# MaxHalford/sorobn

Hardware: NVIDIA H100
Metric: exact-inference queries/sec (higher is better)
Workload: dtype f32

## Files before the change

sorobn_b200/csrc/sbn_api.cu:

```cuda
#include <cuda_runtime.h>

#include <algorithm>
#include <cstdarg>
#include <cstdio>
#include <cstdlib>
#include <cstring>
#include <string>
#include <vector>

#include "sbn_chain.h"
#include "sbn_gibbs.cuh"
#include "sbn_internal.h"
#include "sbn_join.h"
#include "sbn_kernels.cuh"
#include "sbn_launch.h"
#include "sbn_pair.h"
#include "sbn_tma.h"

namespace {

thread_local std::string g_err;

int fail(int code, const char *fmt, ...) {
    char buf[512];
// ... 623 lines not shown
            default: return cudaErrorInvalidValue;
        }
        return cudaGetLastError();
    }
    return sbn_batched_launch(q, grid, stream);
}

cudaError_t launch_normalise(sbn_program *P, float *d_out, int64_t ld_out, int64_t n_rows, cudaStream_t stream) {
    P->launches++;
    const int threads = 256;
    const int64_t grid = (n_rows + threads - 1) / threads;
    if (P->f64)
        sbn_normalise<double><<<static_cast<unsigned>(grid), threads, 0, stream>>>(
            reinterpret_cast<const double *>(P->slots[P->post_slot].ptr), P->ld, P->post_batched, P->Q,
            reinterpret_cast<double *>(d_out), ld_out, static_cast<int>(n_rows), 1e-290,
            reinterpret_cast<double *>(P->d_total));
    else
        sbn_normalise<float><<<static_cast<unsigned>(grid), threads, 0, stream>>>(
            P->slots[P->post_slot].ptr, P->ld, P->post_batched, P->Q, d_out, ld_out, static_cast<int>(n_rows),
            SBN_MIN_TOTAL_F32, P->d_total);
    return cudaGetLastError();
}

inline bool hoisted(const sbn_program *P, const StepDesc &st) { return P->mode == 1 && st.kind == 0; }

inline bool chain_on(const sbn_program *P) {
    return P->use_chain && P->chain_fits && P->use_tiled && !P->use_branches && !P->segments.empty();
}

inline bool pair_on(const sbn_program *P) {
    return P->use_pair && P->use_tiled && !P->use_branches && (!chain_on(P) || P->pairs_avoid_segments) && !P->pairs.empty();
}

inline bool graph_allowed(const sbn_program *P) { return P->use_graph; }

int run_table_steps(sbn_program *P) {
    if (P->mode != 1) return SBN_OK;
    SbnStep q;
    for (const StepDesc &st : P->steps) {
        if (!hoisted(P, st)) continue;
        build_params(P, st, nullptr, 0, 1, &q);
        SBN_CUDA(launch_step(P, st, q, P->stream));
    }
    SBN_CUDA(cudaStreamSynchronize(P->stream));
    P->setup_launches = P->launches;
    P->launches = 0;
    return SBN_OK;
}

inline bool fold_normalise(const sbn_program *P, const StepDesc &st, const SbnStep &q) {
#if !SBN_FOLD_NORMALISE
    (void)P;
    (void)st;
    (void)q;
    return false;
#endif
    static const bool enabled = [] {
        const char *e = getenv("SOROBN_B200_FOLD_NORMALISE");
        return e ? atoi(e) != 0 : true;
    }();
    return enabled && !P->f64 && P->post_batched && st.kind == 1 && q.tile_off != nullptr && q.slab_off == nullptr && st.n_tiles == 1 &&
           st.n_out == P->Q && !sbn_tma_eligible(P, st);
}

int issue_all(sbn_program *P, const uint8_t *d_ev, int64_t ld_ev, int64_t n_rows, float *d_out, int64_t ld_out,
              cudaStream_t stream, cudaEvent_t *events) {
    SbnStep q;
    int k = 0;
    bool folded = false;
    bool skip_second = false;
    for (const StepDesc &st : P->steps) {
        if (events) SBN_CUDA(cudaEventRecord(events[k], stream));
        ++k;
        if (hoisted(P, st)) continue;
        const int seg = chain_on(P) ? P->seg_first[k - 1] : -1;
        if (seg == -2) continue;
        if (seg >= 0) {
            P->launches++;
            SBN_CUDA(sbn_chain_launch(P, *P->segments[seg], d_ev, ld_ev, n_rows, d_out, ld_out, stream));
            continue;
        }
        int pair = pair_on(P) ? P->pair_first[k - 1] : -1;
        if (pair == -2 && !skip_second) pair = -1;
        skip_second = false;
        if (pair == -2) continue;
        if (pair >= 0 && !sbn_pair_fits(P, *P->pairs[pair])) pair = -1;
        if (pair >= 0) {
            skip_second = true;
            P->launches++;
            SBN_CUDA(sbn_pair_launch(P, *P->pairs[pair], d_ev, ld_ev, n_rows, stream));
            continue;
        }
        build_params(P, st, d_ev, ld_ev, n_rows, &q);
        if (k == static_cast<int>(P->steps.size()) && fold_normalise(P, st, q)) {
            q.norm_out = d_out;
            q.norm_ld = ld_out;
            q.norm_totals = P->d_total;
            q.norm_min = SBN_MIN_TOTAL_F32;
            folded = true;
        }
        SBN_CUDA(launch_step(P, st, q, stream));
    }
    if (events) SBN_CUDA(cudaEventRecord(events[k], stream));
    if (!folded && !(chain_on(P) && !P->segments.empty() && P->segments.back()->ends_in_posterior))
        SBN_CUDA(launch_normalise(P, d_out, ld_out, n_rows, stream));
    if (events) SBN_CUDA(cudaEventRecord(events[k + 1], stream));
    return SBN_OK;
// ... 72 lines not shown
}

extern "C" {

int sbn_abi_version(void) { return SBN_ABI_VERSION; }
const char *sbn_last_error(void) { return g_err.c_str(); }

int sbn_device_count(int *count) {
    if (!count) return fail(SBN_E_INVALID, "null count");
    int n = 0;
    cudaError_t e = cudaGetDeviceCount(&n);
    if (e != cudaSuccess || n == 0) {
        *count = 0;
        return fail(SBN_E_NODEVICE, "no CUDA device: %s", cudaGetErrorString(e));
    }
    *count = n;
    return SBN_OK;
}

static int create_common(int device, const int32_t *words, int64_t n_words, const void *tables, int64_t n_table_floats,
                         bool f64, sbn_program **out) {
    if (!words || !out || (n_table_floats > 0 && !tables)) return fail(SBN_E_INVALID, "null argument");
    *out = nullptr;
    sbn_program *P = new sbn_program();
    P->device = device;
    P->f64 = f64;
    {
        const char *e = getenv("SOROBN_B200_CHAIN");
        P->use_chain = e && atoi(e) != 0;
        e = getenv("SOROBN_B200_TMA");
        P->use_tma = e && atoi(e) != 0;
        e = getenv("SOROBN_B200_PAIR");
        P->use_pair = e ? atoi(e) != 0 : true;
    }
    const size_t elem = f64 ? 8 : 4;
    int rc = parse(P, words, n_words);

    if (rc != SBN_OK) {
        delete P;
        return rc;
    }
    for (size_t t = 0; t < P->tables.size(); ++t) {
        if (P->tables[t].first + P->table_padded[t] > n_table_floats) {
            delete P;
            return fail(SBN_E_INVALID, "table %zu lies outside the table blob", t);
        }
    }
    int n_dev = 0;
    if (cudaGetDeviceCount(&n_dev) != cudaSuccess || n_dev == 0) {
        delete P;
        return fail(SBN_E_NODEVICE, "no CUDA device available");
    }
    if (device < 0 || device >= n_dev) {
        delete P;
        return fail(SBN_E_NODEVICE, "device %d out of range (%d visible)", device, n_dev);
    }
    auto bail = [&](int code) {
        sbn_program_destroy(P);
        return code;
    };
#define SBN_CUDA_P(call)                                                                                      \
    do {                                                                                                      \
        cudaError_t e_ = (call);                                                                              \
        if (e_ != cudaSuccess)                                                                                \
            return bail(fail(SBN_E_CUDA, "%s failed: %s (%s:%d)", #call, cudaGetErrorString(e_), __FILE__, __LINE__)); \
    } while (0)
// ... 356 lines not shown
        rc = sbn_program_reserve(P, n_rows);
        if (rc != SBN_OK) return rc;
    }
    if (n_rows > P->reserved_rows) return fail(SBN_E_NOMEM, "n_rows exceeds the scratch that fits the device");
    cudaStream_t stream = static_cast<cudaStream_t>(stream_);
    std::vector<cudaEvent_t> ev(n + 1);
    for (auto &e : ev) SBN_CUDA(cudaEventCreate(&e));
    rc = issue_all(P, d_ev, ld_ev, n_rows, d_out, ld_out, stream, ev.data());
    if (rc == SBN_OK) {
        cudaError_t e = cudaStreamSynchronize(stream);
        if (e != cudaSuccess) rc = fail(SBN_E_CUDA, "profile run failed: %s", cudaGetErrorString(e));
    }
    if (rc == SBN_OK)
        for (int64_t i = 0; i < n; ++i) cudaEventElapsedTime(&step_ms[i], ev[i], ev[i + 1]);
    for (auto &e : ev) cudaEventDestroy(e);
    return rc;
}

int sbn_program_info(const sbn_program *P, int64_t *info, int64_t n_info) {
    if (!P || !info || n_info < 8) return fail(SBN_E_INVALID, "info needs at least 8 entries");
    if (n_info >= 12) {
        int64_t covered = 0, hbm = 0, scratch = 0;
        for (const SbnSegment *seg : P->segments) {
            covered += static_cast<int64_t>(seg->steps.size());
            hbm += seg->hbm_bytes_per_row;
            scratch = std::max(scratch, seg->scratch_floats);
        }
        info[8] = chain_on(P) ? static_cast<int64_t>(P->segments.size()) : 0;
        info[9] = chain_on(P) ? covered : 0;
        info[10] = chain_on(P) ? hbm : 0;
        info[11] = scratch;
    }
    if (n_info >= 14) {
        int64_t saved = 0;
        for (const SbnPair *pr : P->pairs) saved += 8 * P->steps[pr->step1].n_out;
        info[12] = pair_on(P) ? static_cast<int64_t>(P->pairs.size()) : 0;
        info[13] = pair_on(P) ? saved : 0;
    }
    info[0] = P->Q;
    info[1] = P->n_ev;
    info[2] = static_cast<int64_t>(P->steps.size());
    info[3] = batched_floats_per_row(P);
    info[4] = P->reserved_rows;
    info[5] = P->launches;
    info[6] = P->mode;
    int64_t shared = 0;
    for (const Slot &s : P->slots)
        if (!s.batched) shared += s.size;
    info[7] = shared;
    return SBN_OK;
}

int sbn_program_step_roles(const sbn_program *P, int32_t *roles, int64_t n_roles) {
    if (!P || !roles || n_roles < static_cast<int64_t>(P->steps.size())) return fail(SBN_E_INVALID, "roles needs n_steps entries");
    int first_kind = 0;
    bool second_follows = false;
    for (size_t i = 0; i < P->steps.size(); ++i) {
        const StepDesc &st = P->steps[i];
        if (P->mode != 1 || hoisted(P, st)) {
            roles[i] = 0;
            continue;
        }
        roles[i] = 1;
        if (chain_on(P) && P->seg_first[i] != -1) {
            roles[i] = 6;
            continue;
        }
        int pair = pair_on(P) ? P->pair_first[i] : -1;
        if (pair == -2 && !second_follows) pair = -1;
        second_follows = false;
        if (pair == -2) roles[i] = first_kind == 1 ? 5 : 3;
        if (pair >= 0 && sbn_pair_fits(P, *P->pairs[pair])) {
            first_kind = P->pairs[pair]->kind;
            roles[i] = first_kind == 1 ? 4 : 2;
            second_follows = true;
        }
    }
    return SBN_OK;
}

static void drop_graphs(sbn_program *P) {
    if (P->exec) {
        cudaGraphExecDestroy(P->exec);
        P->exec = nullptr;
    }
    if (P->pipe_exec) {
        cudaGraphExecDestroy(P->pipe_exec);
        P->pipe_exec = nullptr;
    }
}

int sbn_program_set_graph(sbn_program *P, int enabled) {
    if (!P) return fail(SBN_E_INVALID, "null program");
    P->use_graph = enabled != 0;
    P->use_branches = enabled == 3;
    drop_graphs(P);
    return SBN_OK;
}

int sbn_program_set_tiled(sbn_program *P, int enabled) {
    if (!P) return fail(SBN_E_INVALID, "null program");
    drop_graphs(P);
    P->use_tiled = enabled != 0;
    P->use_preload = enabled != 4;
    P->use_slab = enabled != 5;
    if (enabled == 8) P->use_tma = false;
    if (enabled == 9) P->use_tma = true;
    if (enabled == 6) P->use_chain = false;
    if (enabled == 7) P->use_chain = true;
    if (enabled == 10) P->use_pair = false;
    if (enabled == 11) P->use_pair = true;
    return SBN_OK;
}

int sbn_host_alloc(void **ptr, int64_t bytes) {
    if (!ptr || bytes <= 0) return fail(SBN_E_INVALID, "bad host allocation request");
    SBN_CUDA(cudaHostAlloc(ptr, static_cast<size_t>(bytes), cudaHostAllocDefault));
    return SBN_OK;
}

int sbn_host_free(void *ptr) {
    if (ptr) SBN_CUDA(cudaFreeHost(ptr));
    return SBN_OK;
}

}

struct sbn_sampler {
    int device = 0;
    int n_vars = 0, n_query = 0, n_ev = 0, n_cycle = 0, Q = 0;
    int32_t *d_ints = nullptr;
    float *d_tables = nullptr;
    const int32_t *card = nullptr, *cpt_off = nullptr, *par_ptr = nullptr, *par_idx = nullptr, *par_stride = nullptr,
                  *chi_ptr = nullptr, *chi_idx = nullptr, *chi_stride = nullptr, *cycle = nullptr, *query = nullptr,
                  *ev_var = nullptr, *prog = nullptr, *flat = nullptr;
    int prog_words = 0, flat_words = 0;
    int64_t table_floats = 0;
    int max_card = 1;
    std::vector<int32_t> h_cycle;
    std::vector<int32_t> h_card;
    uint8_t *d_ev = nullptr;
    float *d_out = nullptr;
    int64_t cap = 0;
    cudaStream_t stream = nullptr;
// ... 350 lines not shown
```

sorobn_b200/csrc/sbn_internal.h:

```cpp
#pragma once
#include <cuda_runtime.h>
#include <stdint.h>

#include <string>
#include <utility>
#include <vector>

#include "../../include/sorobn_b200.h"

struct EvAxis {
    int col, stride, card;
};
struct InDesc {
    bool is_slot;
    int id;
    bool batched;
    int sx;
    std::vector<EvAxis> ev;
    std::vector<int> estrides;
    std::vector<int> strides;
};
struct StepDesc {
    int kind;
    int out_slot;
    int cx;
    int64_t n_out;
    std::vector<int> cards;
    std::vector<int> ecards;
    int64_t zoff_pos = -1;
    int64_t zoff_tiled_pos = -1;
    std::vector<InDesc> in;
    int tile = 0;
    int nu = 0, na = 0, nb = 0, nc = 0;
    std::vector<int> order;
    int64_t n_tiles = 0;
    int64_t tile_off_pos = 0;
    bool slab = false;
    bool big_tables = false;
    int slab_ma = 0, n_slab = 0;
    int64_t slab_off_pos = 0;
    int64_t slab_tile_off_pos = 0;
    int64_t tiles_per_super = 0, n_super = 0;
    int64_t slice_pos = -1;
    int64_t slice_tpc = 0;
    int64_t slice_smem = 0;
};
struct Slot {
    bool batched;
    int64_t size;
    int64_t padded;
    float *ptr;
};

inline int64_t round_up(int64_t v, int64_t m) { return (v + m - 1) / m * m; }

struct SbnSegment;
struct SbnPair;

struct sbn_program {
    int device = 0;
    int n_sms = 1;
    bool f64 = false;
    int mode = 0, n_ev = 0, Q = 0, post_slot = 0, post_batched = 0;
    std::vector<std::pair<int64_t, int64_t>> tables;
    std::vector<int64_t> table_padded;
    float *d_tables = nullptr;
    std::vector<Slot> slots;
    std::vector<StepDesc> steps;

    int64_t reserved_rows = 0;
    int64_t ld = 0;
    float *d_arena = nullptr;
    float *d_shared = nullptr;
    int32_t *d_tile_off = nullptr;
    float *d_total = nullptr;
    uint8_t *d_ev = nullptr;
    float *d_out = nullptr;
    cudaStream_t stream = nullptr;
    static constexpr int kBranches = 4;
    cudaStream_t branch[kBranches] = {nullptr, nullptr, nullptr, nullptr};
    std::vector<cudaEvent_t> step_done;
    std::vector<cudaEvent_t> pipe_events;
    cudaGraphExec_t pipe_exec = nullptr;
    struct {
        const void *ev;
        int64_t ld_ev, n_rows;
        const void *out;
        int64_t ld_out;
    } pipe_key = {nullptr, 0, 0, nullptr, 0};
    int64_t pipe_launches = 0;
    bool use_branches = false;

    bool use_graph = true;
    bool use_tiled = true;
    bool use_slab = true;
    bool use_preload = true;
    cudaGraphExec_t exec = nullptr;
    struct {
        const uint8_t *ev;
        int64_t ld_ev, n_rows;
        float *out;
        int64_t ld_out;
    } graph_key = {nullptr, 0, 0, nullptr, 0};
    int64_t graph_launches = 0;

    int64_t launches = 0;
    int64_t setup_launches = 0;

    std::vector<SbnSegment *> segments;
    std::vector<int> seg_first;
    float *d_chain_scratch = nullptr;
    bool use_chain = true;
    bool use_tma = true;
    bool chain_fits = true;
    std::vector<int32_t> h_tile_words;

    std::vector<SbnPair *> pairs;
    std::vector<int> pair_first;
    float *d_pair_canon = nullptr;
    int32_t *d_pair_tiles = nullptr;
    bool use_pair = true;
    bool pairs_avoid_segments = false;
};
```

sorobn_b200/csrc/sbn_pair.cu:

```cuda
#include "sbn_pair.h"

#include <algorithm>
#include <cstdlib>
#include <cstring>

#include "sbn_internal.h"
#include "sbn_kernels.cuh"
#include "sbn_launch.h"

namespace {

constexpr int kV = 2;

__device__ __forceinline__ void pair_coef8(float (&c)[SBN_PAIR_PW], const float *s) {
    const float4 lo = *reinterpret_cast<const float4 *>(s);
    const float4 hi = *reinterpret_cast<const float4 *>(s + 4);
    c[0] = lo.x, c[1] = lo.y, c[2] = lo.z, c[3] = lo.w;
    c[4] = hi.x, c[5] = hi.y, c[6] = hi.z, c[7] = hi.w;
}

template <int V>
__device__ __forceinline__ void pair_ev_offsets(const SbnPairParams &p, const SbnPairEv &d, int b, int (&e)[V]) {
#pragma unroll
    for (int l = 0; l < V; ++l) e[l] = 0;
    for (int k = 0; k < d.n; ++k) {
        const uint8_t *col = p.ev + static_cast<int64_t>(d.col[k]) * p.ld_ev + b;
#pragma unroll
        for (int l = 0; l < V; ++l) e[l] += ((b + l < p.n_rows) ? min(static_cast<int>(col[l]), d.card[k] - 1) : 0) * d.stride[k];
    }
}

struct PairG {
    const float *p;
    uint32_t base;
    uint32_t x[SBN_PAIR_T], d0[SBN_PAIR_T], d1[SBN_PAIR_T];
};

template <int MODE, int V>
__device__ __forceinline__ void pair_step(const float (&in)[SBN_PAIR_T][SBN_PAIR_T][V], float (&acc)[SBN_PAIR_T][SBN_PAIR_T][V],
                                          const float *k, const int (&e)[V], const PairG &G) {
    constexpr int T = SBN_PAIR_T, PW = SBN_PAIR_PW;
    constexpr bool PACKED = V == 2 && (MODE == SBN_PAIR_CE || MODE == SBN_PAIR_GB || MODE == SBN_PAIR_GC);
#pragma unroll
    for (int d0 = 0; d0 < T; ++d0)
#pragma unroll
        for (int d1 = 0; d1 < T; ++d1)
#pragma unroll
            for (int l = 0; l < V; ++l) acc[d0][d1][l] = 0.f;
#pragma unroll
    for (int x = 0; x < T; ++x) {
        float c[V][PW];
        float cp[T][V];
        if constexpr (MODE == SBN_PAIR_B) {
#pragma unroll
            for (int l = 0; l < V; ++l) pair_coef8(c[l], k + e[l] + x * PW);
        } else if constexpr (MODE == SBN_PAIR_GB) {
#pragma unroll
            for (int d1 = 0; d1 < T; ++d1) sbn_ldv<V>(cp[d1], G.p + (G.base + G.x[x] + G.d1[d1]));
        }
#pragma unroll
        for (int d0 = 0; d0 < T; ++d0) {
            if constexpr (MODE == SBN_PAIR_CU) {
                pair_coef8(c[0], k + (x * T + d0) * PW);
            } else if constexpr (MODE == SBN_PAIR_CE) {
#pragma unroll
                for (int d1 = 0; d1 < T; ++d1)
#pragma unroll
                    for (int l = 0; l < V; ++l) cp[d1][l] = k[e[l] + (x * T + d0) * T + d1];
            } else if constexpr (MODE == SBN_PAIR_GC) {
#pragma unroll
                for (int d1 = 0; d1 < T; ++d1) sbn_ldv<V>(cp[d1], G.p + (G.base + G.x[x] + G.d0[d0] + G.d1[d1]));
            }
#pragma unroll
            for (int d1 = 0; d1 < T; ++d1) {
                if constexpr (PACKED) {
                    sbn_fma2(acc[d0][d1], in[x][d0], cp[d1]);
                } else {
#pragma unroll
                    for (int l = 0; l < V; ++l)
                        acc[d0][d1][l] = fmaf(in[x][d0][l], c[MODE == SBN_PAIR_CU ? 0 : l][d1], acc[d0][d1][l]);
                }
            }
        }
    }
}

template <int M1, int M2>
__global__ void __launch_bounds__(SBN_PAIR_ROWS / kV, (M1 >= SBN_PAIR_GB ? 4 : 5)) sbn_pair_kernel(const __grid_constant__ SbnPairParams p) {
    constexpr int T = SBN_PAIR_T, V = kV;
    extern __shared__ __align__(16) float s_canon[];
    __shared__ __align__(8) uint64_t s_bar;
    sbn_pdl_launch_dependents();

    const int rblock = blockIdx.x / p.n_chunks;
    const int chunk = blockIdx.x % p.n_chunks;
    if (threadIdx.x == 0) {
        sbn_mbar_init(&s_bar, 1);
        sbn_fence_mbar_init();
    }
    __syncthreads();
    if (threadIdx.x == 0) {
        sbn_mbar_expect_tx(&s_bar, static_cast<uint32_t>(p.canon_floats) * 4u);
        sbn_tma_bulk_g2s(s_canon, p.canon, static_cast<uint32_t>(p.canon_floats) * 4u, &s_bar);
    }
// ... 46 lines not shown
        for (int x = 0; x < T; ++x)
#pragma unroll
            for (int y = 0; y < T; ++y) sbn_ldv<V>(f[x][y], fp + (fb + xs[x] + ys[y]));
        if (p.has_pre1) {
            const float *const k = s_canon + r1.x;
#pragma unroll
            for (int x = 0; x < T; ++x)
#pragma unroll
                for (int y = 0; y < T; ++y)
#pragma unroll
                    for (int l = 0; l < V; ++l) f[x][y][l] *= k[g1[l] + x * T + y];
        }
        float mid[T][T][V];
        if constexpr (M1 == SBN_PAIR_GB || M1 == SBN_PAIR_GC) G.base = static_cast<uint32_t>(r1.z) * ld;
        pair_step<M1, V>(f, mid, s_canon + r0.z, e1, G);
        if (p.has_pre2) {
            const float *const k = s_canon + r1.y;
#pragma unroll
            for (int y = 0; y < T; ++y)
#pragma unroll
                for (int w = 0; w < T; ++w)
#pragma unroll
                    for (int l = 0; l < V; ++l) mid[y][w][l] *= k[g2[l] + y * T + w];
        }
        float acc[T][T][V];
        pair_step<M2, V>(mid, acc, s_canon + r0.w, e2, G);

#pragma unroll
        for (int z = 0; z < T; ++z)
#pragma unroll
            for (int w = 0; w < T; ++w)
                if (w < p.cw && z < p.cz) sbn_stv<V>(op + (ob + ow[w] + oz[z]), acc[w][z]);
    }
}

template <int MINB>
__global__ void __launch_bounds__(SBN_TRIPLE_THREADS, MINB) sbn_triple_kernel(const __grid_constant__ SbnTripleParams p) {
    constexpr int T = SBN_PAIR_T;
    sbn_pdl_entry();
    const int rblock = blockIdx.x / p.n_chunks;
    const int chunk = blockIdx.x % p.n_chunks;
    const int b = rblock * static_cast<int>(blockDim.x) + threadIdx.x;
    if (b >= p.n_rows) return;
    const uint32_t ld = static_cast<uint32_t>(p.ld);
    const int g = threadIdx.y;
    const float *const ap = p.a + b + static_cast<uint32_t>(g * p.a_g) * ld;
    const float *const bp = p.b + b;
    const float *const cp = p.c + b;
    float *const op = p.out + b + static_cast<uint32_t>(g * p.o_g) * ld;
    uint32_t ak[T], aj[T], bj[T], bs[T], ck[T], cz[T];
#pragma unroll
    for (int d = 0; d < T; ++d) {
        ak[d] = static_cast<uint32_t>(d * p.a_k) * ld, aj[d] = static_cast<uint32_t>(d * p.a_j) * ld;
        bj[d] = static_cast<uint32_t>(d * p.b_j) * ld, bs[d] = static_cast<uint32_t>(d * p.b_s) * ld;
        ck[d] = static_cast<uint32_t>(d * p.c_k) * ld, cz[d] = static_cast<uint32_t>(d * p.c_z) * ld;
    }
    const uint32_t oz = static_cast<uint32_t>(p.o_z) * ld, os = static_cast<uint32_t>(p.o_s) * ld;
    const int t_begin = chunk * p.tiles_per_cta;
    const int t_end = min(p.n_tiles, t_begin + p.tiles_per_cta);
    for (int t = t_begin; t < t_end; ++t) {
        const int4 row = __ldg(reinterpret_cast<const int4 *>(p.tile_off) + t);
        float acc[T][T];
#pragma unroll
        for (int z = 0; z < T; ++z)
#pragma unroll
            for (int s = 0; s < T; ++s) acc[z][s] = 0.f;
// ... 288 lines not shown
    q.c_k = C.estrides[kk], q.c_p = C.estrides[1 - kk], q.c_z = C.strides[kz];
    int64_t os = 1;
    std::vector<int64_t> os2(n2);
    for (int k = 0; k < n2; ++k) os2[k] = os, os *= s2.cards[k];
    q.o_z = static_cast<int32_t>(os2[kz]);
    q.o_s = static_cast<int32_t>(os2[ks]);
    q.group = kg >= 0 ? T : 1;
    q.o_g = kg >= 0 ? static_cast<int32_t>(os2[kg]) : 0;
    q.a_g = kg >= 0 ? A.strides[to1[kg]] : 0;
    std::vector<int> dig(r2.size(), 0);
    for (int64_t t = 0; t < n_tiles; ++t) {
        int64_t ob = 0, ab = 0, bb = 0, cb = 0;
        for (size_t k = 0; k < r2.size(); ++k) {
            const int ax = r2[k];
            ob += dig[k] * os2[ax];
            cb += static_cast<int64_t>(dig[k]) * C.strides[ax];
            if (to1[ax] >= 0) {
                ab += static_cast<int64_t>(dig[k]) * A.strides[to1[ax]];
                bb += static_cast<int64_t>(dig[k]) * B.strides[to1[ax]];
            }
        }
        tiles->push_back(static_cast<int32_t>(ob));
        tiles->push_back(static_cast<int32_t>(ab));
        tiles->push_back(static_cast<int32_t>(bb));
        tiles->push_back(static_cast<int32_t>(cb));
        for (size_t k = 0; k < dig.size(); ++k) {
            if (++dig[k] < s2.cards[r2[k]]) break;
            dig[k] = 0;
        }
    }
    return pr;
}

}

cudaError_t sbn_pair_set_attrs() {
    return cudaSuccess;
}

void sbn_pair_free(sbn_program *P) {
    for (SbnPair *pr : P->pairs) delete pr;
    P->pairs.clear();
    P->pair_first.clear();
    cudaFree(P->d_pair_canon);
    cudaFree(P->d_pair_tiles);
    P->d_pair_canon = nullptr;
    P->d_pair_tiles = nullptr;
}

cudaError_t sbn_pair_plan(sbn_program *P) {
    constexpr int T = SBN_PAIR_T;
    P->pair_first.assign(P->steps.size(), -1);
    if (P->mode != 1 || P->f64) return cudaSuccess;
    static const int min_card = [] {
        const char *e = getenv("SOROBN_B200_PAIR_MIN_CARD");
        return e ? atoi(e) : 4;
    }();

    static const bool triples_on = [] {
        const char *e = getenv("SOROBN_B200_TRIPLE");
        return e ? atoi(e) != 0 : true;
    }();

    HostTables H;
    std::vector<float> canon;
    std::vector<int32_t> tiles;
    cudaError_t err = cudaSuccess;
    bool fetched = false;

    const int n_steps = static_cast<int>(P->steps.size());
    auto launched = [&](int i) { return P->steps[i].kind != 0; };
    P->pairs_avoid_segments = P->use_chain && !P->segments.empty();
    auto in_segment = [&](int i) { return P->pairs_avoid_segments && P->seg_first[i] != -1; };
    for (int i1 = 0; i1 < n_steps; ++i1) {
        if (!launched(i1) || P->pair_first[i1] != -1) continue;
        int i2 = i1 + 1;
        while (i2 < n_steps && !launched(i2)) ++i2;
        if (i2 >= n_steps) break;
        if (in_segment(i1) || in_segment(i2)) continue;
        const StepDesc &s1 = P->steps[i1], &s2 = P->steps[i2];
        if (triples_on) {
            if (SbnPair *tr = plan_triple(P, i1, i2, &tiles)) {
                P->pair_first[i1] = static_cast<int>(P->pairs.size());
                P->pair_first[i2] = -2;
                P->pairs.push_back(tr);
// ... 71 lines not shown
            SbnPair *pr = new SbnPair();
            memset(&pr->q, 0, sizeof pr->q);
            memset(&pr->t, 0, sizeof pr->t);
            pr->kind = 0;
            pr->step1 = i1, pr->step2 = i2, pr->f_in = fi, pr->g_in = gi;
            pr->m1 = mode_of(c1.layout), pr->m2 = mode_of(c2.layout);
            if (gi >= 0) pr->m1 = s1.in[gi].strides[jy] == 0 ? SBN_PAIR_GB : SBN_PAIR_GC;
            pr->canon_pos = static_cast<int64_t>(canon.size());
            pr->tile_off_pos = static_cast<int64_t>(tiles.size());
            SbnPairParams &q = pr->q;
            q.canon_floats = static_cast<int32_t>(total);
            const int64_t at_c1 = 0, at_c2 = c1.floats(), at_g1 = at_c2 + c2.floats(), at_g2 = at_g1 + g1.floats();
            canon.resize(canon.size() + static_cast<size_t>(total), 0.f);
            fill_canon(c1, canon.data() + pr->canon_pos + at_c1);
            fill_canon(c2, canon.data() + pr->canon_pos + at_c2);
            fill_canon(g1, canon.data() + pr->canon_pos + at_g1);
            fill_canon(g2, canon.data() + pr->canon_pos + at_g2);
            q.n_tiles = static_cast<int32_t>(n_tiles);
            q.f_sx = F.estrides[0];
            q.f_sy = F.strides[jy];
            q.cx = cx, q.cy = cy, q.cw = s2.cards[kw], q.cz = s2.cards[kz];
            int64_t os = 1;
            std::vector<int64_t> os2(n2);
            for (int k = 0; k < n2; ++k) os2[k] = os, os *= s2.cards[k];
            q.o_sw = static_cast<int32_t>(os2[kw]);
            q.o_sz = static_cast<int32_t>(os2[kz]);
            if (gi >= 0) q.g_x = s1.in[gi].estrides[0], q.g_y = s1.in[gi].strides[jy], q.g_w = s1.in[gi].strides[jw];
            q.has_pre1 = g1.tabs.empty() ? 0 : 1;
            q.has_pre2 = g2.tabs.empty() ? 0 : 1;
            set_ev(&q.ev_main1, c1);
            set_ev(&q.ev_main2, c2);
            set_ev(&q.ev_pre1, g1);
            set_ev(&q.ev_pre2, g2);
            std::vector<int> dig(r2.size(), 0);
            for (int64_t t = 0; t < n_tiles; ++t) {
                int64_t ob = 0, fb = 0;
                for (size_t k = 0; k < r2.size(); ++k) {
                    ob += dig[k] * os2[r2[k]];
                    fb += static_cast<int64_t>(dig[k]) * F.strides[r1[k]];
                }
                tiles.push_back(static_cast<int32_t>(ob));
                tiles.push_back(static_cast<int32_t>(fb));
                tiles.push_back(static_cast<int32_t>(at_c1 + tile_slab(c1, r1, dig)));
                tiles.push_back(static_cast<int32_t>(at_c2 + tile_slab(c2, r2, dig)));
                tiles.push_back(static_cast<int32_t>(at_g1 + tile_slab(g1, r1, dig)));
                tiles.push_back(static_cast<int32_t>(at_g2 + tile_slab(g2, r2, dig)));
                int64_t gb = 0;
                if (gi >= 0)
                    for (size_t k = 0; k < r1.size(); ++k) gb += static_cast<int64_t>(dig[k]) * s1.in[gi].strides[r1[k]];
                tiles.push_back(static_cast<int32_t>(gb));
                tiles.push_back(0);
                for (size_t k = 0; k < dig.size(); ++k) {
                    if (++dig[k] < s2.cards[r2[k]]) break;
                    dig[k] = 0;
                }
            }
            P->pair_first[i1] = static_cast<int>(P->pairs.size());
            P->pair_first[i2] = -2;
            P->pairs.push_back(pr);
            break;
        }
    }
    if (P->pairs.empty()) return cudaSuccess;
    err = cudaMalloc(&P->d_pair_canon, std::max<size_t>(canon.size(), 4) * 4);
    if (err != cudaSuccess) return err;
    err = cudaMalloc(&P->d_pair_tiles, tiles.size() * 4);
    if (err != cudaSuccess) return err;
    if (!canon.empty()) err = cudaMemcpy(P->d_pair_canon, canon.data(), canon.size() * 4, cudaMemcpyHostToDevice);
    if (err != cudaSuccess) return err;
    return cudaMemcpy(P->d_pair_tiles, tiles.data(), tiles.size() * 4, cudaMemcpyHostToDevice);
}

static cudaError_t triple_launch(sbn_program *P, const SbnPair &pr, int64_t n_rows, cudaStream_t stream) {
    SbnTripleParams q = pr.t;
    const StepDesc &s1 = P->steps[pr.step1], &s2 = P->steps[pr.step2];
    q.a = P->slots[s1.in[pr.a_in].id].ptr;
    q.b = P->slots[s1.in[pr.b_in].id].ptr;
    q.c = P->slots[s2.in[pr.c_in].id].ptr;
    q.out = P->slots[s2.out_slot].ptr;
    q.ld = P->ld;
    q.n_rows = static_cast<int32_t>(n_rows);
    q.tile_off = P->d_pair_tiles + pr.tile_off_pos;
    const int rows_per_cta = q.group > 1 ? 32 : 128;
    const int64_t n_rblocks = (n_rows + rows_per_cta - 1) / rows_per_cta;
    static const int64_t tpc_env = [] {
        const char *e = getenv("SOROBN_B200_TRIPLE_TPC");
        return e ? atoll(e) : 1LL;
    }();
    static const int minb = [] {
        const char *e = getenv("SOROBN_B200_TRIPLE_MINB");
        return e ? atoi(e) : 3;
    }();
    const int64_t tpc = std::max<int64_t>(1, std::min<int64_t>(q.n_tiles, tpc_env));
    q.tiles_per_cta = static_cast<int32_t>(tpc);
    q.n_chunks = static_cast<int32_t>((q.n_tiles + tpc - 1) / tpc);
    const int64_t grid = q.n_chunks * n_rblocks;
    if (grid >= (1LL << 31)) return cudaErrorInvalidConfiguration;
    const dim3 g(static_cast<unsigned>(grid)), b(rows_per_cta, q.group);
    if (minb == 3) sbn_launch(sbn_triple_kernel<3>, g, b, 0, stream, q);
    else if (minb == 1) sbn_launch(sbn_triple_kernel<1>, g, b, 0, stream, q);
    else sbn_launch(sbn_triple_kernel<2>, g, b, 0, stream, q);
    return cudaGetLastError();
}

bool sbn_pair_fits(const sbn_program *P, const SbnPair &pr) {
    const StepDesc &s1 = P->steps[pr.step1], &s2 = P->steps[pr.step2];
    int64_t entries = P->slots[s2.out_slot].size;
    for (const InDesc &in : s1.in)
        if (in.batched) entries = std::max(entries, P->slots[in.id].size);
    for (const InDesc &in : s2.in)
        if (in.batched && in.id != s1.out_slot) entries = std::max(entries, P->slots[in.id].size);
    const char *e = getenv("SOROBN_B200_PAIR_IDX_LIMIT");
    const int64_t limit = e ? atoll(e) : (1LL << 31);
    return entries * P->ld < limit;
}

cudaError_t sbn_pair_launch(sbn_program *P, const SbnPair &pr, const uint8_t *d_ev, int64_t ld_ev, int64_t n_rows,
                            cudaStream_t stream) {
    if (pr.kind == 1) return triple_launch(P, pr, n_rows, stream);
    SbnPairParams q = pr.q;
    const StepDesc &s1 = P->steps[pr.step1], &s2 = P->steps[pr.step2];
    q.f = P->slots[s1.in[pr.f_in].id].ptr;
    q.g = pr.g_in >= 0 ? P->slots[s1.in[pr.g_in].id].ptr : q.f;
    q.out = P->slots[s2.out_slot].ptr;
    q.ev = d_ev;
    q.ld_ev = ld_ev;
    q.ld = P->ld;
    q.n_rows = static_cast<int32_t>(n_rows);
    q.canon = P->d_pair_canon + pr.canon_pos;
    q.tile_off = P->d_pair_tiles + pr.tile_off_pos;
    const int64_t n_rblocks = (n_rows + SBN_PAIR_ROWS - 1) / SBN_PAIR_ROWS;
    static const int64_t target_env = [] {
        const char *e = getenv("SOROBN_B200_PAIR_CTAS");
        return e ? atoll(e) : 0LL;
    }();
    const int64_t target = target_env > 0 ? target_env : 8LL * P->n_sms * 6;
    const int64_t chunks = std::max<int64_t>(1, std::min<int64_t>(q.n_tiles, target / std::max<int64_t>(1, n_rblocks)));
    const int64_t tpc = (q.n_tiles + chunks - 1) / chunks;
    q.tiles_per_cta = static_cast<int32_t>(tpc);
    q.n_chunks = static_cast<int32_t>((q.n_tiles + tpc - 1) / tpc);
    const int64_t grid = q.n_chunks * n_rblocks;
    if (grid >= (1LL << 31)) return cudaErrorInvalidConfiguration;
    launch_modes(pr, q, static_cast<unsigned>(grid), static_cast<size_t>(q.canon_floats) * 4, stream);
    return cudaGetLastError();
}
```

sorobn_b200/csrc/sbn_pair.h:

```cpp
#pragma once
#include <cuda_runtime.h>
#include <stdint.h>

#include <vector>

#include "../../include/sorobn_b200.h"

#define SBN_PAIR_T 5
#define SBN_PAIR_PW 8
#define SBN_PAIR_MAX_EV 4
#define SBN_PAIR_ROWS 256
#define SBN_TRIPLE_THREADS 160
#define SBN_PAIR_SMEM_MAX (40 * 1024)

struct SbnPairEv {
    int32_t n;
    int32_t col[SBN_PAIR_MAX_EV], stride[SBN_PAIR_MAX_EV], card[SBN_PAIR_MAX_EV];
};

struct SbnPairParams {
    const float *f;
    float *out;
    const uint8_t *ev;
    const float *canon;
    const int32_t *tile_off;
    int64_t ld_ev, ld;
    int32_t n_rows;
    int32_t canon_floats;
    int32_t n_tiles, tiles_per_cta, n_chunks;
    int32_t f_sx, f_sy;
    int32_t cx, cy, cw, cz;
    int32_t o_sw, o_sz;
    int32_t has_pre1, has_pre2;
    SbnPairEv ev_main1, ev_main2, ev_pre1, ev_pre2;
    const float *g;
    int32_t g_x, g_y, g_w;
};

enum SbnPairMode { SBN_PAIR_B = 0, SBN_PAIR_CU = 1, SBN_PAIR_CE = 2, SBN_PAIR_GB = 3, SBN_PAIR_GC = 4 };

struct SbnTripleParams {
    const float *a, *b, *c;
    float *out;
    const int32_t *tile_off;
    int64_t ld;
    int32_t n_rows;
    int32_t n_tiles, tiles_per_cta, n_chunks;
    int32_t a_p, a_k, a_j;
    int32_t b_p, b_j, b_s;
    int32_t c_p, c_k, c_z;
    int32_t o_z, o_s;
    int32_t group;
    int32_t a_g, o_g;
};

struct SbnPair {
    int kind;
    int step1, step2;
    int f_in;
    int g_in;
    int m1, m2;
    SbnPairParams q;
    SbnTripleParams t;
    int a_in, b_in, c_in;
    int64_t tile_off_pos;
    int64_t canon_pos;
};

struct sbn_program;
cudaError_t sbn_pair_plan(sbn_program *P);
cudaError_t sbn_pair_launch(sbn_program *P, const SbnPair &pr, const uint8_t *d_ev, int64_t ld_ev, int64_t n_rows,
                            cudaStream_t stream);
bool sbn_pair_fits(const sbn_program *P, const SbnPair &pr);
cudaError_t sbn_pair_set_attrs();
void sbn_pair_free(sbn_program *P);
```

Measured before the change: 23.34 million.

## Fuse chains of consecutive pair steps into a single register-resident run kernel

Adds a planner that finds chains of up to three consecutive pair launches where each pair's output feeds only the next pair, with matching tile shapes and a tile-to-tile mapping. It packs their canonical coefficient blocks per tile into one contiguous buffer that is loaded into shared memory with a bulk copy. A new kernel then runs all the pair steps while keeping the intermediate factor in registers. This removes the HBM round trips for intermediates and the per-pair launch overhead, at the cost of a larger register footprint, more shared memory per block and runtime mode dispatch inside the kernel. It only engages when there are at least twice the SM count times the per-block row count.

```diff
diff --git a/sorobn_b200/csrc/sbn_api.cu b/sorobn_b200/csrc/sbn_api.cu
--- a/sorobn_b200/csrc/sbn_api.cu
+++ b/sorobn_b200/csrc/sbn_api.cu
@@ -679,6 +679,10 @@
     return P->use_pair && P->use_tiled && !P->use_branches && (!chain_on(P) || P->pairs_avoid_segments) && !P->pairs.empty();
 }
 
+inline bool run_engaged(const sbn_program *P, int64_t n_rows) {
+    return pair_on(P) && P->use_run && !P->runs.empty() && n_rows >= 2LL * P->n_sms * SBN_PAIR_ROWS;
+}
+
 inline bool graph_allowed(const sbn_program *P) { return P->use_graph; }
 
 int run_table_steps(sbn_program *P) {
@@ -716,10 +720,21 @@
     int k = 0;
     bool folded = false;
     bool skip_second = false;
+    P->issued_rows = n_rows;
+    const bool runs = run_engaged(P, n_rows);
+    int run_last = -1;
     for (const StepDesc &st : P->steps) {
         if (events) SBN_CUDA(cudaEventRecord(events[k], stream));
         ++k;
         if (hoisted(P, st)) continue;
+        if (k - 1 <= run_last) continue;
+        const int run = runs ? P->run_first[k - 1] : -1;
+        if (run >= 0 && sbn_run_fits(P, *P->runs[run])) {
+            run_last = P->runs[run]->step_last;
+            P->launches++;
+            SBN_CUDA(sbn_run_launch(P, *P->runs[run], d_ev, ld_ev, n_rows, stream));
+            continue;
+        }
         const int seg = chain_on(P) ? P->seg_first[k - 1] : -1;
         if (seg == -2) continue;
         if (seg >= 0) {
@@ -858,6 +873,8 @@
         P->use_tma = e && atoi(e) != 0;
         e = getenv("SOROBN_B200_PAIR");
         P->use_pair = e ? atoi(e) != 0 : true;
+        e = getenv("SOROBN_B200_RUN");
+        P->use_run = e ? atoi(e) != 0 : true;
     }
     const size_t elem = f64 ? 8 : 4;
     int rc = parse(P, words, n_words);
@@ -1280,9 +1297,15 @@
         info[11] = scratch;
     }
     if (n_info >= 14) {
-        int64_t saved = 0;
-        for (const SbnPair *pr : P->pairs) saved += 8 * P->steps[pr->step1].n_out;
-        info[12] = pair_on(P) ? static_cast<int64_t>(P->pairs.size()) : 0;
+        int64_t saved = 0, fewer = 0;
+        for (const SbnPair *pr : P->pairs) saved += 8 * P->steps[pr->step1].n_out, ++fewer;
+        if (run_engaged(P, P->issued_rows))
+            for (const SbnRun *run : P->runs) {
+                if (!sbn_run_fits(P, *run)) continue;
+                fewer += run->n_pairs - 1;
+                for (int j = run->pair0; j + 1 < run->pair0 + run->n_pairs; ++j) saved += 8 * P->steps[P->pairs[j]->step2].n_out;
+            }
+        info[12] = pair_on(P) ? fewer : 0;
         info[13] = pair_on(P) ? saved : 0;
     }
     info[0] = P->Q;
@@ -1303,6 +1326,8 @@
     if (!P || !roles || n_roles < static_cast<int64_t>(P->steps.size())) return fail(SBN_E_INVALID, "roles needs n_steps entries");
     int first_kind = 0;
     bool second_follows = false;
+    const bool runs = run_engaged(P, P->issued_rows);
+    int run_last = -1;
     for (size_t i = 0; i < P->steps.size(); ++i) {
         const StepDesc &st = P->steps[i];
         if (P->mode != 1 || hoisted(P, st)) {
@@ -1312,6 +1337,16 @@
         roles[i] = 1;
         if (chain_on(P) && P->seg_first[i] != -1) {
             roles[i] = 6;
+            continue;
+        }
+        if (static_cast<int>(i) <= run_last) {
+            roles[i] = 8;
+            continue;
+        }
+        const int run = runs ? P->run_first[i] : -1;
+        if (run >= 0 && sbn_run_fits(P, *P->runs[run])) {
+            roles[i] = 7;
+            run_last = P->runs[run]->step_last;
             continue;
         }
         int pair = pair_on(P) ? P->pair_first[i] : -1;
@@ -1358,6 +1393,8 @@
     if (enabled == 7) P->use_chain = true;
     if (enabled == 10) P->use_pair = false;
     if (enabled == 11) P->use_pair = true;
+    if (enabled == 12) P->use_run = false;
+    if (enabled == 13) P->use_run = true;
     return SBN_OK;
 }
 
diff --git a/sorobn_b200/csrc/sbn_internal.h b/sorobn_b200/csrc/sbn_internal.h
--- a/sorobn_b200/csrc/sbn_internal.h
+++ b/sorobn_b200/csrc/sbn_internal.h
@@ -56,6 +56,7 @@
 
 struct SbnSegment;
 struct SbnPair;
+struct SbnRun;
 
 struct sbn_program {
     int device = 0;
@@ -121,4 +122,8 @@
     int32_t *d_pair_tiles = nullptr;
     bool use_pair = true;
     bool pairs_avoid_segments = false;
+    std::vector<SbnRun *> runs;
+    std::vector<int> run_first;
+    bool use_run = true;
+    int64_t issued_rows = 0;
 };
diff --git a/sorobn_b200/csrc/sbn_pair.cu b/sorobn_b200/csrc/sbn_pair.cu
--- a/sorobn_b200/csrc/sbn_pair.cu
+++ b/sorobn_b200/csrc/sbn_pair.cu
@@ -3,6 +3,7 @@
 #include <algorithm>
 #include <cstdlib>
 #include <cstring>
+#include <unordered_map>
 
 #include "sbn_internal.h"
 #include "sbn_kernels.cuh"
@@ -19,8 +20,8 @@
     c[4] = hi.x, c[5] = hi.y, c[6] = hi.z, c[7] = hi.w;
 }
 
-template <int V>
-__device__ __forceinline__ void pair_ev_offsets(const SbnPairParams &p, const SbnPairEv &d, int b, int (&e)[V]) {
+template <int V, class Params>
+__device__ __forceinline__ void pair_ev_offsets(const Params &p, const SbnPairEv &d, int b, int (&e)[V]) {
 #pragma unroll
     for (int l = 0; l < V; ++l) e[l] = 0;
     for (int k = 0; k < d.n; ++k) {
@@ -34,11 +35,17 @@
     const float *p;
     uint32_t base;
     uint32_t x[SBN_PAIR_T], d0[SBN_PAIR_T], d1[SBN_PAIR_T];
+    __device__ __forceinline__ uint32_t at(int x_, int d0_, int d1_) const { return base + x[x_] + d0[d0_] + d1[d1_]; }
 };
-
-template <int MODE, int V>
+struct RunG {
+    const float *p;
+    uint32_t base, sx, s0, s1;
+    __device__ __forceinline__ uint32_t at(int x_, int d0_, int d1_) const { return base + x_ * sx + d0_ * s0 + d1_ * s1; }
+};
+
+template <int MODE, int V, class GT = PairG>
 __device__ __forceinline__ void pair_step(const float (&in)[SBN_PAIR_T][SBN_PAIR_T][V], float (&acc)[SBN_PAIR_T][SBN_PAIR_T][V],
-                                          const float *k, const int (&e)[V], const PairG &G) {
+                                          const float *k, const int (&e)[V], const GT &G) {
     constexpr int T = SBN_PAIR_T, PW = SBN_PAIR_PW;
     constexpr bool PACKED = V == 2 && (MODE == SBN_PAIR_CE || MODE == SBN_PAIR_GB || MODE == SBN_PAIR_GC);
 #pragma unroll
@@ -56,7 +63,7 @@
             for (int l = 0; l < V; ++l) pair_coef8(c[l], k + e[l] + x * PW);
         } else if constexpr (MODE == SBN_PAIR_GB) {
 #pragma unroll
-            for (int d1 = 0; d1 < T; ++d1) sbn_ldv<V>(cp[d1], G.p + (G.base + G.x[x] + G.d1[d1]));
+            for (int d1 = 0; d1 < T; ++d1) sbn_ldv<V>(cp[d1], G.p + G.at(x, 0, d1));
         }
 #pragma unroll
         for (int d0 = 0; d0 < T; ++d0) {
@@ -69,7 +76,7 @@
                     for (int l = 0; l < V; ++l) cp[d1][l] = k[e[l] + (x * T + d0) * T + d1];
             } else if constexpr (MODE == SBN_PAIR_GC) {
 #pragma unroll
-                for (int d1 = 0; d1 < T; ++d1) sbn_ldv<V>(cp[d1], G.p + (G.base + G.x[x] + G.d0[d0] + G.d1[d1]));
+                for (int d1 = 0; d1 < T; ++d1) sbn_ldv<V>(cp[d1], G.p + G.at(x, d0, d1));
             }
 #pragma unroll
             for (int d1 = 0; d1 < T; ++d1) {
@@ -182,6 +189,96 @@
             for (int w = 0; w < T; ++w)
                 if (w < p.cw && z < p.cz) sbn_stv<V>(op + (ob + ow[w] + oz[z]), acc[w][z]);
     }
+}
+
+template <bool HAS_G>
+__device__ __forceinline__ void run_step(const SbnRunParams &p, int s, int b, int t, const float *blk, float (&in)[SBN_PAIR_T][SBN_PAIR_T][kV],
+                                         float (&acc)[SBN_PAIR_T][SBN_PAIR_T][kV]) {
+    constexpr int T = SBN_PAIR_T, V = kV;
+    const SbnRunStep &st = p.st[s];
+    if (st.has_pre) {
+        int g[V];
+        pair_ev_offsets<V>(p, st.ev_pre, b, g);
+        const float *const k = blk + st.pre_off;
+#pragma unroll
+        for (int x = 0; x < T; ++x)
+#pragma unroll
+            for (int y = 0; y < T; ++y)
+#pragma unroll
+                for (int l = 0; l < V; ++l) in[x][y][l] *= k[g[l] + x * T + y];
+    }
+    int e[V];
+    pair_ev_offsets<V>(p, st.ev_main, b, e);
+    const float *const k = blk + st.main_off;
+    RunG G;
+    G.p = nullptr;
+    G.base = G.sx = G.s0 = G.s1 = 0;
+    switch (st.mode) {
+        case SBN_PAIR_B: pair_step<SBN_PAIR_B, V>(in, acc, k, e, G); break;
+        case SBN_PAIR_CU: pair_step<SBN_PAIR_CU, V>(in, acc, k, e, G); break;
+        case SBN_PAIR_CE: pair_step<SBN_PAIR_CE, V>(in, acc, k, e, G); break;
+        default: {
+            if constexpr (!HAS_G) break;
+            const int j = s / 2;
+            const uint32_t ld = static_cast<uint32_t>(p.ld);
+            G.p = p.g[j] + b;
+            G.base = static_cast<uint32_t>(__ldg(p.tile_off + 8 * t + 2 + j)) * ld;
+            G.sx = static_cast<uint32_t>(p.g_x[j]) * ld;
+            G.s0 = static_cast<uint32_t>(p.g_y[j]) * ld;
+            G.s1 = static_cast<uint32_t>(p.g_w[j]) * ld;
+            if (st.mode == SBN_PAIR_GB) pair_step<SBN_PAIR_GB, V>(in, acc, k, e, G);
+            else pair_step<SBN_PAIR_GC, V>(in, acc, k, e, G);
+        }
+    }
+}
+
+template <bool HAS_G>
+__global__ void __launch_bounds__(SBN_PAIR_ROWS / kV, HAS_G ? 3 : 4) sbn_run_kernel(const __grid_constant__ SbnRunParams p) {
+    constexpr int T = SBN_PAIR_T, V = kV;
+    extern __shared__ __align__(16) float s_blk[];
+    __shared__ __align__(8) uint64_t s_bar;
+    sbn_pdl_launch_dependents();
+
+    const int rblock = blockIdx.x / p.n_tiles;
+    const int t = blockIdx.x % p.n_tiles;
+    if (threadIdx.x == 0) {
+        sbn_mbar_init(&s_bar, 1);
+        sbn_fence_mbar_init();
+    }
+    __syncthreads();
+    if (threadIdx.x == 0) {
+        sbn_mbar_expect_tx(&s_bar, static_cast<uint32_t>(p.block_floats) * 4u);
+        sbn_tma_bulk_g2s(s_blk, p.canon + static_cast<int64_t>(t) * p.block_floats, static_cast<uint32_t>(p.block_floats) * 4u, &s_bar);
+    }
+    const int b = (rblock * static_cast<int>(blockDim.x) + threadIdx.x) * V;
+    const bool live = b < p.n_rows;
+    sbn_mbar_wait(&s_bar, 0);
+    if (!live) return;
+    sbn_pdl_wait();
+
+    const uint32_t ld = static_cast<uint32_t>(p.ld);
+    const uint32_t fb = static_cast<uint32_t>(__ldg(p.tile_off + 8 * t + 1)) * ld;
+    const float *const fp = p.f + b;
+    float f[T][T][V];
+#pragma unroll
+    for (int x = 0; x < T; ++x)
+#pragma unroll
+        for (int y = 0; y < T; ++y)
+            sbn_ldv<V>(f[x][y], fp + (fb + static_cast<uint32_t>(min(x, p.cx - 1) * p.f_sx) * ld + static_cast<uint32_t>(min(y, p.cy - 1) * p.f_sy) * ld));
+    float mid[T][T][V];
+#pragma unroll 1
+    for (int j = 0; j < p.n_pairs; ++j) {
+        run_step<HAS_G>(p, 2 * j, b, t, s_blk, f, mid);
+        run_step<false>(p, 2 * j + 1, b, t, s_blk, mid, f);
+    }
+    const uint32_t ob = static_cast<uint32_t>(__ldg(p.tile_off + 8 * t)) * ld;
+    float *const op = p.out + b;
+#pragma unroll
+    for (int z = 0; z < T; ++z)
+#pragma unroll
+        for (int w = 0; w < T; ++w)
+            if (w < p.cw && z < p.cz)
+                sbn_stv<V>(op + (ob + static_cast<uint32_t>(w * p.o_sw) * ld + static_cast<uint32_t>(z * p.o_sz) * ld), f[w][z]);
 }
 
 template <int MINB>
@@ -536,6 +633,140 @@
     return pr;
 }
 
+bool sole_reader(const sbn_program *P, int writer, int reader) {
+    const int slot = P->steps[writer].out_slot;
+    for (int i = writer + 1; i < static_cast<int>(P->steps.size()); ++i) {
+        for (const InDesc &in : P->steps[i].in)
+            if (in.is_slot && in.id == slot && i != reader) return false;
+        if (P->steps[i].out_slot == slot) break;
+    }
+    return true;
+}
+
+bool pairs_chain(const sbn_program *P, const SbnPair &a, const SbnPair &b, const std::vector<int32_t> &tiles,
+                 std::vector<int64_t> *next_tile) {
+    if (a.kind != 0 || b.kind != 0) return false;
+    int next = a.step2 + 1;
+    while (next < static_cast<int>(P->steps.size()) && P->steps[next].kind == 0) ++next;
+    if (next != b.step1) return false;
+    const StepDesc &a2 = P->steps[a.step2], &b1 = P->steps[b.step1];
+    const InDesc &F = b1.in[b.f_in];
+    if (!F.is_slot || F.id != a2.out_slot || a2.out_slot == P->post_slot || !sole_reader(P, a.step2, b.step1)) return false;
+    if (b.q.cx != a.q.cw || b.q.cy != a.q.cz || b.q.f_sx != a.q.o_sw || b.q.f_sy != a.q.o_sz || b.q.n_tiles != a.q.n_tiles)
+        return false;
+    std::unordered_map<int32_t, int64_t> reader;
+    for (int64_t t = 0; t < b.q.n_tiles; ++t) reader.emplace(tiles[b.tile_off_pos + 8 * t + 1], t);
+    if (static_cast<int64_t>(reader.size()) != b.q.n_tiles) return false;
+    next_tile->assign(a.q.n_tiles, -1);
+    for (int64_t t = 0; t < a.q.n_tiles; ++t) {
+        const auto it = reader.find(tiles[a.tile_off_pos + 8 * t]);
+        if (it == reader.end()) return false;
+        (*next_tile)[t] = it->second;
+    }
+    return true;
+}
+
+int64_t run_block_floats(const sbn_program *P, int p0, int n) {
+    const SbnPair &first = *P->pairs[p0], &last = *P->pairs[p0 + n - 1];
+    const int out = P->steps[last.step2].out_slot;
+    int64_t blk = 0;
+    for (int j = p0; j < p0 + n; ++j) {
+        const SbnPair &pr = *P->pairs[j];
+        if (pr.g_in >= 0 && P->steps[pr.step1].in[pr.g_in].id == out) return -1;
+        for (int a = 0; a < 4; ++a) blk += round_up(pr.n_e[a] * pr.slab[a], 4);
+    }
+    return blk * 4 <= SBN_PAIR_SMEM_MAX ? blk : -1;
+}
+
+void plan_runs(sbn_program *P, std::vector<float> *canon, std::vector<int32_t> *tiles) {
+    P->run_first.assign(P->steps.size(), -1);
+    const int n_pairs = static_cast<int>(P->pairs.size());
+    for (int p0 = 0; p0 < n_pairs;) {
+        int n = 1;
+        std::vector<int64_t> next[SBN_RUN_MAX_PAIRS];
+        while (p0 + n < n_pairs && n < SBN_RUN_MAX_PAIRS && pairs_chain(P, *P->pairs[p0 + n - 1], *P->pairs[p0 + n], *tiles, &next[n - 1]) &&
+               run_block_floats(P, p0, n + 1) >= 0)
+            ++n;
+        const SbnPair &first = *P->pairs[p0], &last = *P->pairs[p0 + n - 1];
+        if (n >= 2 && P->steps[first.step1].in[first.f_in].id == P->steps[last.step2].out_slot) {
+            std::vector<int64_t> all;
+            bool ok = true;
+            for (int64_t t = 0; t < first.q.n_tiles && ok; ++t) {
+                int64_t tl = t;
+                for (int j = 1; j < n; ++j) tl = next[j - 1][tl];
+                std::vector<int64_t> rd, wr;
+                const int64_t fb = (*tiles)[first.tile_off_pos + 8 * t + 1], ob = (*tiles)[last.tile_off_pos + 8 * tl];
+                for (int x = 0; x < first.q.cx; ++x)
+                    for (int y = 0; y < first.q.cy; ++y) rd.push_back(fb + x * first.q.f_sx + y * first.q.f_sy);
+                for (int w = 0; w < last.q.cw; ++w)
+                    for (int z = 0; z < last.q.cz; ++z) wr.push_back(ob + w * last.q.o_sw + z * last.q.o_sz);
+                std::sort(rd.begin(), rd.end());
+                std::sort(wr.begin(), wr.end());
+                ok = rd == wr;
+                all.insert(all.end(), rd.begin(), rd.end());
+            }
+            std::sort(all.begin(), all.end());
+            if (!ok || std::adjacent_find(all.begin(), all.end()) != all.end()) n = 1;
+        }
+        if (n < 2) {
+            ++p0;
+            continue;
+        }
+        const int64_t blk = run_block_floats(P, p0, n);
+        SbnRun *run = new SbnRun();
+        memset(&run->q, 0, sizeof run->q);
+        run->pair0 = p0, run->n_pairs = n;
+        run->step_first = first.step1, run->step_last = last.step2;
+        SbnRunParams &q = run->q;
+        const int64_t n_tiles = first.q.n_tiles;
+        q.block_floats = static_cast<int32_t>(blk);
+        q.n_tiles = static_cast<int32_t>(n_tiles);
+        q.n_pairs = n;
+        q.f_sx = first.q.f_sx, q.f_sy = first.q.f_sy, q.cx = first.q.cx, q.cy = first.q.cy;
+        q.cw = last.q.cw, q.cz = last.q.cz, q.o_sw = last.q.o_sw, q.o_sz = last.q.o_sz;
+        int64_t off[SBN_RUN_MAX_PAIRS][4], at = 0;
+        for (int j = 0; j < n; ++j) {
+            const SbnPair &pr = *P->pairs[p0 + j];
+            for (int a = 0; a < 4; ++a) off[j][a] = at, at += round_up(pr.n_e[a] * pr.slab[a], 4);
+            q.g_x[j] = pr.q.g_x, q.g_y[j] = pr.q.g_y, q.g_w[j] = pr.q.g_w;
+            const SbnPairEv *evs[4] = {&pr.q.ev_main1, &pr.q.ev_main2, &pr.q.ev_pre1, &pr.q.ev_pre2};
+            for (int h = 0; h < 2; ++h) {
+                SbnRunStep &s = q.st[2 * j + h];
+                s.mode = h == 0 ? pr.m1 : pr.m2;
+                s.has_pre = h == 0 ? pr.q.has_pre1 : pr.q.has_pre2;
+                s.main_off = static_cast<int32_t>(off[j][h]);
+                s.pre_off = static_cast<int32_t>(off[j][h + 2]);
+                s.ev_main = *evs[h];
+                s.ev_pre = *evs[h + 2];
+                for (int k = 0; k < s.ev_main.n; ++k) s.ev_main.stride[k] /= static_cast<int32_t>(pr.n_r[h]);
+                for (int k = 0; k < s.ev_pre.n; ++k) s.ev_pre.stride[k] /= static_cast<int32_t>(pr.n_r[h + 2]);
+            }
+        }
+        run->canon_pos = static_cast<int64_t>(canon->size());
+        canon->resize(canon->size() + static_cast<size_t>(n_tiles * blk), 0.f);
+        run->tile_off_pos = static_cast<int64_t>(tiles->size());
+        for (int64_t t = 0; t < n_tiles; ++t) {
+            int64_t tj[SBN_RUN_MAX_PAIRS] = {t, 0, 0};
+            for (int j = 1; j < n; ++j) tj[j] = next[j - 1][tj[j - 1]];
+            for (int j = 0; j < n; ++j) {
+                const SbnPair &pr = *P->pairs[p0 + j];
+                for (int a = 0; a < 4; ++a) {
+                    const int64_t src = pr.canon_pos + (*tiles)[pr.tile_off_pos + 8 * tj[j] + 2 + a];
+                    float *dst = canon->data() + run->canon_pos + t * blk + off[j][a];
+                    for (int64_t e = 0; e < pr.n_e[a]; ++e)
+                        std::copy_n(canon->data() + src + e * pr.n_r[a] * pr.slab[a], pr.slab[a], dst + e * pr.slab[a]);
+                }
+            }
+            int32_t row[8] = {(*tiles)[last.tile_off_pos + 8 * tj[n - 1]], (*tiles)[first.tile_off_pos + 8 * t + 1], 0, 0, 0, 0, 0, 0};
+            for (int j = 0; j < n; ++j) row[2 + j] = (*tiles)[P->pairs[p0 + j]->tile_off_pos + 8 * tj[j] + 6];
+            tiles->insert(tiles->end(), row, row + 8);
+        }
+        P->run_first[run->step_first] = static_cast<int>(P->runs.size());
+        P->runs.push_back(run);
+        p0 += n;
+    }
+}
+
 }
 
 cudaError_t sbn_pair_set_attrs() {
@@ -544,8 +775,11 @@
 
 void sbn_pair_free(sbn_program *P) {
     for (SbnPair *pr : P->pairs) delete pr;
+    for (SbnRun *run : P->runs) delete run;
     P->pairs.clear();
     P->pair_first.clear();
+    P->runs.clear();
+    P->run_first.clear();
     cudaFree(P->d_pair_canon);
     cudaFree(P->d_pair_tiles);
     P->d_pair_canon = nullptr;
@@ -555,6 +789,7 @@
 cudaError_t sbn_pair_plan(sbn_program *P) {
     constexpr int T = SBN_PAIR_T;
     P->pair_first.assign(P->steps.size(), -1);
+    P->run_first.assign(P->steps.size(), -1);
     if (P->mode != 1 || P->f64) return cudaSuccess;
     static const int min_card = [] {
         const char *e = getenv("SOROBN_B200_PAIR_MIN_CARD");
@@ -692,6 +927,13 @@
             set_ev(&q.ev_main2, c2);
             set_ev(&q.ev_pre1, g1);
             set_ev(&q.ev_pre2, g2);
+            {
+                int a = 0;
+                for (const CanonSpec *cs : {&c1, &c2, &g1, &g2}) {
+                    pr->slab[a] = cs->slab, pr->n_r[a] = cs->n_r, pr->n_e[a] = cs->tabs.empty() ? 0 : cs->n_e;
+                    ++a;
+                }
+            }
             std::vector<int> dig(r2.size(), 0);
             for (int64_t t = 0; t < n_tiles; ++t) {
                 int64_t ob = 0, fb = 0;
@@ -722,6 +964,7 @@
         }
     }
     if (P->pairs.empty()) return cudaSuccess;
+    plan_runs(P, &canon, &tiles);
     err = cudaMalloc(&P->d_pair_canon, std::max<size_t>(canon.size(), 4) * 4);
     if (err != cudaSuccess) return err;
     err = cudaMalloc(&P->d_pair_tiles, tiles.size() * 4);
@@ -775,6 +1018,37 @@
     return entries * P->ld < limit;
 }
 
+bool sbn_run_fits(const sbn_program *P, const SbnRun &run) {
+    for (int j = run.pair0; j < run.pair0 + run.n_pairs; ++j)
+        if (!sbn_pair_fits(P, *P->pairs[j])) return false;
+    return true;
+}
+
+cudaError_t sbn_run_launch(sbn_program *P, const SbnRun &run, const uint8_t *d_ev, int64_t ld_ev, int64_t n_rows,
+                           cudaStream_t stream) {
+    SbnRunParams q = run.q;
+    const SbnPair &first = *P->pairs[run.pair0];
+    q.f = P->slots[P->steps[first.step1].in[first.f_in].id].ptr;
+    q.out = P->slots[P->steps[run.step_last].out_slot].ptr;
+    for (int j = 0; j < run.n_pairs; ++j) {
+        const SbnPair &pr = *P->pairs[run.pair0 + j];
+        q.g[j] = pr.g_in >= 0 ? P->slots[P->steps[pr.step1].in[pr.g_in].id].ptr : q.f;
+    }
+    q.ev = d_ev;
+    q.ld_ev = ld_ev;
+    q.ld = P->ld;
+    q.n_rows = static_cast<int32_t>(n_rows);
+    q.canon = P->d_pair_canon + run.canon_pos;
+    q.tile_off = P->d_pair_tiles + run.tile_off_pos;
+    const int64_t grid = static_cast<int64_t>(q.n_tiles) * ((n_rows + SBN_PAIR_ROWS - 1) / SBN_PAIR_ROWS);
+    if (grid >= (1LL << 31)) return cudaErrorInvalidConfiguration;
+    bool has_g = false;
+    for (int j = 0; j < run.n_pairs; ++j) has_g = has_g || P->pairs[run.pair0 + j]->g_in >= 0;
+    sbn_launch(has_g ? sbn_run_kernel<true> : sbn_run_kernel<false>, dim3(static_cast<unsigned>(grid)), dim3(SBN_PAIR_ROWS / kV), static_cast<size_t>(q.block_floats) * 4,
+               stream, q);
+    return cudaGetLastError();
+}
+
 cudaError_t sbn_pair_launch(sbn_program *P, const SbnPair &pr, const uint8_t *d_ev, int64_t ld_ev, int64_t n_rows,
                             cudaStream_t stream) {
     if (pr.kind == 1) return triple_launch(P, pr, n_rows, stream);
diff --git a/sorobn_b200/csrc/sbn_pair.h b/sorobn_b200/csrc/sbn_pair.h
--- a/sorobn_b200/csrc/sbn_pair.h
+++ b/sorobn_b200/csrc/sbn_pair.h
@@ -54,6 +54,31 @@
     int32_t a_g, o_g;
 };
 
+#define SBN_RUN_MAX_PAIRS 3
+
+struct SbnRunStep {
+    int32_t mode, has_pre;
+    int32_t main_off, pre_off;
+    SbnPairEv ev_main, ev_pre;
+};
+
+struct SbnRunParams {
+    const float *f;
+    float *out;
+    const uint8_t *ev;
+    const float *canon;
+    const int32_t *tile_off;
+    int64_t ld_ev, ld;
+    int32_t n_rows;
+    int32_t block_floats;
+    int32_t n_tiles, n_pairs;
+    int32_t f_sx, f_sy, cx, cy;
+    int32_t cw, cz, o_sw, o_sz;
+    const float *g[SBN_RUN_MAX_PAIRS];
+    int32_t g_x[SBN_RUN_MAX_PAIRS], g_y[SBN_RUN_MAX_PAIRS], g_w[SBN_RUN_MAX_PAIRS];
+    SbnRunStep st[2 * SBN_RUN_MAX_PAIRS];
+};
+
 struct SbnPair {
     int kind;
     int step1, step2;
@@ -65,6 +90,14 @@
     int a_in, b_in, c_in;
     int64_t tile_off_pos;
     int64_t canon_pos;
+    int64_t slab[4], n_r[4], n_e[4];
+};
+
+struct SbnRun {
+    int pair0, n_pairs;
+    int step_first, step_last;
+    SbnRunParams q;
+    int64_t tile_off_pos, canon_pos;
 };
 
 struct sbn_program;
@@ -72,5 +105,8 @@
 cudaError_t sbn_pair_launch(sbn_program *P, const SbnPair &pr, const uint8_t *d_ev, int64_t ld_ev, int64_t n_rows,
                             cudaStream_t stream);
 bool sbn_pair_fits(const sbn_program *P, const SbnPair &pr);
+bool sbn_run_fits(const sbn_program *P, const SbnRun &run);
+cudaError_t sbn_run_launch(sbn_program *P, const SbnRun &run, const uint8_t *d_ev, int64_t ld_ev, int64_t n_rows,
+                           cudaStream_t stream);
 cudaError_t sbn_pair_set_attrs();
 void sbn_pair_free(sbn_program *P);
```

After: 25.22 million (median of 6 runs). +8.1%, better.
